# phantomzone-org/fhe-ram

Hardware: AMD Instinct MI355X
Metric: encrypted RAM read ops/s + write ops/s at 2^18 entries; achieved HBM GB/s vs peak (higher is better)
Workload: dtype f64

## Files before the change

fhe-ram_amd/csrc/ctx.hpp:

```cpp
#pragma once
#include "../../include/fheram.h"
#include "kernels.hpp"
#include "cmux_chain.hpp"

#include <algorithm>
#include <atomic>
#include <cstdio>
#include <cstdlib>
#include <cstring>
#include <map>
#include <string>
#include <vector>

using namespace fk;

namespace {

thread_local std::string g_create_err;


struct ProfCls {
    uint64_t launches = 0, blocks = 0;
    double ms = 0.0;
    std::vector<std::pair<hipEvent_t, hipEvent_t>> pending;
};

}

inline uint64_t next_addr_id() { static std::atomic<uint64_t> n{0}; return ++n; }

struct RamState {
    bool initialized = false, state = false;
    bool memo_top = false;
    int memo_alone = 0;
    bool res_in_trtop = false;
};

struct fheram_ctx {
    fheram_params p;
    int device = 0;
    hipStream_t stream = nullptr;
    hipStream_t stream2 = nullptr;
    hipStream_t cur = nullptr;
    hipEvent_t ev_fork = nullptr, ev_join = nullptr;
    hipEvent_t ev_xout = nullptr, ev_xin = nullptr;
    bool side_begun = false;
    bool trhi_in_C = false;
    bool tree_rotate_pending = false;
    int ws = 0, n2 = 0, n_digits = 0;
    size_t rows = 0;
    size_t rows_glob = 0;
    int shard = 0, n_shards = 1;
    std::vector<std::vector<int>> base2d;
    static constexpr int S_CT = 3, S_ADDR = 4, S_INV = 5, DNUM_CT = 3, DNUM_GGSW = 4;
    int s_evk = 4;
    size_t atk = 0;
    static constexpr size_t GLWE = (size_t)S_CT * 2 * N;
    static constexpr size_t GLWE4 = (size_t)S_ADDR * 2 * N;
    static constexpr size_t GGSW = (size_t)DNUM_CT * 2 * GLWE4;
    static constexpr size_t EVK5 = (size_t)DNUM_GGSW * S_INV * 2 * N;
    static constexpr size_t GGSW5 = (size_t)DNUM_GGSW * 2 * S_INV * 2 * N;
    double* d_tw = nullptr;
    double ninv = 0.0;
    double* d_atk = nullptr;
    double* d_atk_inv = nullptr;
    double* d_tsk = nullptr;
    int64_t gal[LOGN];
    bool keys_loaded = false;
    int32_t* d_data = nullptr;
    int32_t* d_tree = nullptr;
    int32_t* d_scrA = nullptr;
    int32_t* d_scrB = nullptr;
    int32_t* d_scrC = nullptr;
    int32_t* d_scrD = nullptr;
    int32_t* d_res = nullptr;
    int32_t* d_tmp = nullptr;
    int32_t* d_tmp2 = nullptr;
    int32_t* d_w = nullptr;
    double* d_big = nullptr;
    double* d_big2 = nullptr;
    int limb_split = 1;
    int chain = 1;
    int chain_y = 3;
    int fine_split = 1;
    int use_graph = 0;
    int32_t* d_part = nullptr;
    int32_t* d_gat[3] = {nullptr, nullptr, nullptr};
    int nco = 0;
    int cus = 256;
    double* d_prep = nullptr;
    bool prep1_ready = false;
    int32_t* d_ggsw_tmp = nullptr;
    int32_t* d_ggsw_tmp2 = nullptr;
    int max_digits = 0;
    RamState ram;
    bool words_staged = false;
    int memo = 1;
    int tail = 1;
    int tail_ep = 1;
    int tail_test = 0;
    unsigned tail_seq = 0;
    int tail_xoff = 0;
    uint64_t tail_launches = 0;
    unsigned* h_tail_fb = nullptr;
    unsigned tail_fb_mark = 0;
    uint64_t tail_launch_mark = 0;
    unsigned* d_tail_sync = nullptr;
    int mid = 2;
    int mid_test = 0;
    unsigned mid_seq = 0;
    uint64_t mid_launches = 0, mid_launch_mark = 0;
    unsigned mid_fb_mark = 0;
    int mid_bad_windows = 0, mid_saved = 0;
    uint64_t mid_window_cts = 0, mid_disabled_count = 0;
    unsigned mid_off_ops = 0;
    unsigned* h_mid_fb = nullptr;
    unsigned* d_mid_sync[2] = {nullptr, nullptr};
    double* d_mid_big[2] = {nullptr, nullptr};
    double* d_mid_y[2] = {nullptr, nullptr};
    int pair_z = 1;
    int fuse = 1;
    bool wide = false;
    int safe = 0;
    int monitor = 1;
    unsigned* h_ro_flag = nullptr;
    int pre_inv = 1;
    uint64_t inv_id[2] = {0, 0};
    double* d_prep_inv = nullptr;
    int32_t* d_ggsw_inv = nullptr;
    hipEvent_t ev_inv[2] = {nullptr, nullptr};
// ... 193 lines not shown
```

fhe-ram_amd/csrc/kernels.hpp:

```cpp
#pragma once
#include "fft_dev.hpp"
#include <type_traits>

namespace fk {

#ifdef FK_STAMP
__device__ unsigned long long g_stamps[192];
#define STAMP(i)                                                                                   \
    do {                                                                                           \
        __builtin_amdgcn_sched_barrier(0);                                                         \
        if (threadIdx.x == 0 && blockIdx.x == 0 && blockIdx.y == 0 && blockIdx.z == 0) {           \
            unsigned long long t_;                                                                 \
            asm volatile("s_memtime %0\n\ts_waitcnt lgkmcnt(0)" : "=s"(t_)::"memory");            \
            g_stamps[i] = t_;                                                                      \
        }                                                                                          \
        __builtin_amdgcn_sched_barrier(0);                                                         \
    } while (0)
#define STAMPZ(i)                                                                                  \
    do {                                                                                           \
        __builtin_amdgcn_sched_barrier(0);                                                         \
        if (threadIdx.x == 0 && blockIdx.x == 0 && blockIdx.y == 0 && (blockIdx.z == 0 || blockIdx.z == 3)) { \
            unsigned long long t_;                                                                 \
            asm volatile("s_memtime %0\n\ts_waitcnt lgkmcnt(0)" : "=s"(t_)::"memory");            \
            g_stamps[(blockIdx.z == 0 ? 128 : 144) + (i)] = t_;                                      \
// ... 1322 lines not shown
                bstage[tid + T * k] = window51(__builtin_floor(__builtin_fma(aa[k] - ab[k], 0.5, 0.5)));
                u[k] = window51(__builtin_floor(__builtin_fma(aa[k] + ab[k], 0.5, 0.5)));
            }
        }
    }
    twiddles_commit(twr, tw, tid);
    double xh[SX][E];
    double od[E], ec[E];
    {
        int sidx = sidx0;
#pragma unroll
        for (int k = 0; k < E; k++) {
            const bool ng = sidx >= N;
            double c = mstage[sidx & (N - 1)];
            const double d2 = take_digit(c);
            const double d1 = take_digit(c);
            const double d0 = cmod17(c);
            xh[2][k] = ng ? -d2 : d2;
            xh[1][k] = ng ? -d1 : d1;
            xh[0][k] = ng ? -d0 : d0;
            double w = 0.0;
            if (co == 0) { const double b = bstage[sidx & (N - 1)]; w = ng ? -b : b; }
            od[k] = w;
            ec[k] = 0.0;
            sidx = (sidx + sstep) & (2 * N - 1);
        }
    }
    OpRegs g[SX];
#pragma unroll
    for (int r = 0; r < SX; r++) load_ops(g[r], ka.key + (long)((r * SK + (SK - 1)) * 2 + co) * N, tid);
    fwd_all<SX>(xh, tw, data, tid);
    auto pair = [&](int j) {
        double acc[2][E];
#pragma unroll
        for (int k = 0; k < E; k++) { acc[0][k] = 0.0; acc[1][k] = 0.0; }
#pragma unroll
        for (int r = 0; r < SX; r++) {
            mac_regs(acc[0], xh[r], g[r]);
            __builtin_amdgcn_sched_barrier(0);
            load_ops(g[r], ka.key + (long)((r * SK + (j - 1)) * 2 + co) * N, tid);
            __builtin_amdgcn_sched_barrier(0);
        }
#pragma unroll
        for (int r = 0; r < SX; r++) mac_regs(acc[1], xh[r], g[r]);
        __builtin_amdgcn_sched_barrier(0);
        ntt_inv2_loop(acc, tw, data, data + LDS_DATA, tid);
        fold_limb<SK>(od, ec, acc[0], j);
        fold_limb<SK>(od, ec, acc[1], j - 1);
        if (j >= 2) {
#pragma unroll
            for (int r = 0; r < SX; r++) load_ops(g[r], ka.key + (long)((r * SK + (j - 2)) * 2 + co) * N, tid);
        }
    };
#pragma unroll 1
    for (int j = SK - 1; j >= 1; j -= 2) pair(j);
    if constexpr (SK & 1) {
        double acc[1][E];
#pragma unroll
        for (int k = 0; k < E; k++) acc[0][k] = 0.0;
#pragma unroll
        for (int r = 0; r < SX; r++) mac_regs(acc[0], xh[r], g[r]);
        ntt_inv1_loop(acc, tw, data, tid);
        fold_limb<SK>(od, ec, acc[0], 0);
    }
#pragma unroll
    for (int k = 0; k < E; k++) {
        double r_ = window51(u[k] - window51(od[k]));
        const double d2 = take_digit(r_);
        const double d1 = take_digit(r_);
        int dst = tid + T * k + ka.t;
        const bool ng = dst >= N;
        if (ng) dst -= N;
        gstore_i32(op + glwe_off(2, co), (unsigned)dst * 4u, cneg((int)d2, ng));
        gstore_i32(op + glwe_off(1, co), (unsigned)dst * 4u, cneg((int)d1, ng));
        gstore_i32(op + glwe_off(0, co), (unsigned)dst * 4u, cneg((int)r_, ng));
    }
}

struct RowChainArgs {
    EpChainArgs ep;
    KsChainArgs ks;
    GlweRef hi, trhi;
    int store_ep = 0;
};
#define FK_READ_CHAIN_ARGS RowChainArgs
#define FK_READ_CHAIN_BATCH 0
#define FK_KS_CHAIN_NAME k_keyswitch_chain
#define FK_READ_CHAIN_NAME k_read_chain
#define FK_VG FK_CHAIN_VGPRS
#include "chain_kernels.inc"
#undef FK_KS_CHAIN_NAME
#undef FK_READ_CHAIN_NAME
#undef FK_VG
#define FK_KS_CHAIN_NAME k_keyswitch_chain_w
#define FK_READ_CHAIN_NAME k_read_chain_w
#define FK_VG FK_WIDE_VGPRS
#include "chain_kernels.inc"
#undef FK_KS_CHAIN_NAME
#undef FK_READ_CHAIN_NAME
#undef FK_VG
#undef FK_READ_CHAIN_ARGS
#undef FK_READ_CHAIN_BATCH
struct RowChainBatchArgs : RowChainArgs {
    long opnd_stride = 0;
    int ws = 1, src_rows = 1;
};
template <typename Args>
__device__ __forceinline__ long batch_opnd_offset(const Args& ra) {
    int y = (int)blockIdx.y;
    asm volatile("" : "+v"(y));
    return (long)(__builtin_amdgcn_readfirstlane(y) / ra.ws) * ra.opnd_stride;
}
__device__ __forceinline__ GlweRef batch_src_row(GlweRef a, const RowChainBatchArgs& ra) {
    int y = (int)blockIdx.y;
    asm volatile("" : "+v"(y));
    y = __builtin_amdgcn_readfirstlane(y);
    a.p += (long)(y % ra.src_rows - y) * a.sy;
    return a;
}
#define FK_READ_CHAIN_ARGS RowChainBatchArgs
#define FK_READ_CHAIN_BATCH 1
#define FK_READ_CHAIN_NAME k_read_chain_b
#define FK_VG FK_CHAIN_VGPRS
#include "chain_kernels.inc"
#undef FK_READ_CHAIN_NAME
#undef FK_VG
#define FK_READ_CHAIN_NAME k_read_chain_bw
#define FK_VG FK_WIDE_VGPRS
#include "chain_kernels.inc"
#undef FK_READ_CHAIN_NAME
#undef FK_VG
#undef FK_READ_CHAIN_ARGS
#undef FK_READ_CHAIN_BATCH
struct RowChainListArgs : RowChainArgs {
    long opnd_stride = 0;
    int ws = 1;
    unsigned src_map = 0;
};
__device__ __forceinline__ GlweRef list_src_row(GlweRef a, const RowChainListArgs& ra) {
    int y = (int)blockIdx.y;
    asm volatile("" : "+v"(y));
    const int k = __builtin_amdgcn_readfirstlane(y) / ra.ws;
    const int m = (int)((ra.src_map >> (4 * k)) & 15u);
    a.p += (long)((m - k) * ra.ws) * a.sy;
    return a;
}
#define FK_READ_CHAIN_ARGS RowChainListArgs
#define FK_READ_CHAIN_BATCH 2
#define FK_READ_CHAIN_NAME k_read_chain_lw
#define FK_VG FK_WIDE_VGPRS
#include "chain_kernels.inc"
#undef FK_READ_CHAIN_NAME
#undef FK_VG
#undef FK_READ_CHAIN_ARGS
#undef FK_READ_CHAIN_BATCH

#define FK_WRITE_CHAIN_ARGS RowChainArgs
#define FK_WRITE_CHAIN_BATCH 0
#define FK_WRITE_CHAIN_NAME k_write_chain
#include "write_chain.inc"
#undef FK_WRITE_CHAIN_ARGS
#undef FK_WRITE_CHAIN_BATCH
#undef FK_WRITE_CHAIN_NAME
#define FK_WRITE_CHAIN_ARGS RowChainBatchArgs
#define FK_WRITE_CHAIN_BATCH 1
#define FK_WRITE_CHAIN_NAME k_write_chain_b
// ... 759 lines not shown
```

fhe-ram_amd/csrc/launch.hpp:

```cpp
#pragma once
#include "ctx.hpp"

namespace {

template <typename F>
void with_evk(const fheram_ctx* c, F&& f) {
    if (c->s_evk == 5) f(std::integral_constant<int, 5>{});
    else f(std::integral_constant<int, 4>{});
}
template <typename F>
void with_evk_wide(fheram_ctx* c, bool wide, F&& f) {
    if (wide) c->wide_unsynced = true;
    with_evk(c, [&](auto sk) { if (wide) f(sk, std::true_type{}); else f(sk, std::false_type{}); });
}
bool capturing(const fheram_ctx* c) { return c->use_graph && !c->profile; }

constexpr int LIMB_SPLIT_MAX = 64;
constexpr int EW_SLICES = 8;
int pick_nco(const fheram_ctx* c, int gx, int gy, bool one_wg = false) {
    if (c->nco != 0) return c->nco;
    if (one_wg) return 2;
    return ((long)gx * gy * 2 <= c->cus) ? 1 : 2;
}
void launch_prepare(fheram_ctx* c, const int32_t* in, double* out, int npoly, int64_t gal = 0) {
// ... 207 lines not shown
    if (d >= 2) hipLaunchKernelGGL((k_ext_product_chain_r<4>), dim3(gx, gy, 1), dim3(T), LDS_BYTES, c->cur, ca);
    else hipLaunchKernelGGL((k_ext_product_chain<3, 4>), dim3(gx, gy, 1), dim3(T), LDS_BYTES, c->cur, ca);
}
void ep_chain(fheram_ctx* c, GlweRef src, GlweRef dst, GlweRef tmp, const double* prep, int d, int gx, int gy) {
    if (gx <= 0 || gy <= 0) return;
    GlweRef b[2];
    bool fits;
    switch (plan_chain(c, ChainQuery{true, d, gx, gy}, src, dst, tmp, b, fits).form) {
    case ChainForm::Mid: launch_mid_ep(c, src, b, prep, d, gx, gy); return;
    case ChainForm::Chain:
        if (!fits && !chain_bufs(d, src, tmp, dst, b)) break;
        launch_ep_chain(c, src, b, prep, d, gx, gy);
        if (!fits) launch_copy(c, tmp, dst, gx, gy);
        return;
    default: break;
    }
    run_chain(c, d, src, dst, tmp, gx, gy, [&](int i, GlweRef in, GlweRef out) { launch_ep(c, in, out, prep + (size_t)i * fheram_ctx::GGSW, gx, gy); });
}
void launch_trace_chain(fheram_ctx* c, GlweRef src, const GlweRef (&b)[2], int start, int n, int gx, int gy, int rot_mul, int rot_base) {
    ProfScope ps(c, "keyswitch", (uint64_t)gx * gy, n);
    ProfScope pf(c, "keyswitch_fused", (uint64_t)gx * gy, n);
    ProfScope pl(c, "keyswitch_chain_launch", (uint64_t)gx * gy * n, 1);
    KsChainArgs ca;
    ca.base = ks_args(c, src, src, b[0], trace_key(c, start), c->gal[start], 0, rot_mul, rot_base);
    ca.buf[0] = b[0]; ca.buf[1] = b[1]; ca.n = n;
    for (int i = 0; i < n; i++) { ca.key[i] = trace_key(c, start + i); ca.ginv[i] = galois_inv_mod(galois_mod(c->gal[start + i])); }
    const int yf = n >= 2 ? c->chain_y : 0;
    with_evk_wide(c, yf && c->wide, [&](auto sk, auto w) {
        constexpr int SK = decltype(sk)::value;
        if (!yf) hipLaunchKernelGGL((k_keyswitch_chain<3, SK, 3>), dim3(gx, gy, 1), dim3(T), LDS_BYTES, c->cur, ca);
        else if constexpr (decltype(w)::value) hipLaunchKernelGGL((k_keyswitch_chain_w<3, SK, 3, 3>), dim3(gx, gy, 1), dim3(T), LDS_BYTES, c->cur, ca);
        else hipLaunchKernelGGL((k_keyswitch_chain<3, SK, 3, 3>), dim3(gx, gy, 1), dim3(T), LDS_BYTES, c->cur, ca);
    });
}
struct OpndTable { int ws = 0; long stride = 0; int src_rows = 0; bool mapped = false; unsigned src_map = 0; };
bool use_row_fuse(const fheram_ctx* c, int d, int n_tr, int gx, int gy, bool one_wg = false) {
    return c->fuse && c->chain_y == 3 && !capturing(c) &&
           chain_form(c, ChainQuery{true, d, gx, gy, false, one_wg}).form == ChainForm::Chain &&
           chain_form(c, ChainQuery{false, n_tr, gx, gy, false, one_wg}).form == ChainForm::Chain;
}
RowChainBatchArgs with_table(const RowChainArgs& ra, const OpndTable& t, int src_rows) {
    RowChainBatchArgs rb;
    static_cast<RowChainArgs&>(rb) = ra;
    rb.opnd_stride = t.stride; rb.ws = t.ws; rb.src_rows = src_rows;
    return rb;
}
void fill_row_chain(fheram_ctx* c, RowChainArgs& ra, const double* prep, int d, int start, int n_tr) {
    ra.ep.tw = c->d_tw; ra.ep.n = d;
    for (int i = 0; i < d; i++) ra.ep.ggsw[i] = prep + (size_t)i * fheram_ctx::GGSW;
    ra.ks.n = n_tr;
    for (int i = 0; i < n_tr; i++) { ra.ks.key[i] = trace_key(c, start + i); ra.ks.ginv[i] = galois_inv_mod(galois_mod(c->gal[start + i])); }
}
void launch_read_chain(fheram_ctx* c, GlweRef src, const GlweRef* ep_store, GlweRef dst, const double* prep, int d, int n_tr, int gx, int gy, const OpndTable& t) {
    ProfScope ps(c, "read_chain_launch", (uint64_t)gx * gy, 1);
    RowChainArgs ra;
    fill_row_chain(c, ra, prep, d, 0, n_tr);
    ra.ep.src = src;
    ra.ep.buf[0] = ra.ep.buf[1] = ep_store ? *ep_store : dst;
    ra.store_ep = ep_store ? 1 : 0;
    ra.ks.base = ks_args(c, dst, dst, dst, trace_key(c, 0), c->gal[0]);
    ra.ks.buf[0] = ra.ks.buf[1] = dst;
    ra.hi = dst; ra.trhi = dst;
    if (t.mapped) {
        RowChainListArgs rl;
        static_cast<RowChainArgs&>(rl) = ra;
        rl.opnd_stride = t.stride; rl.ws = t.ws; rl.src_map = t.src_map;
        c->wide_unsynced = true;
        with_evk(c, [&](auto sk) { hipLaunchKernelGGL((k_read_chain_lw<decltype(sk)::value, 4>), dim3(gx, gy, 1), dim3(T), LDS_BYTES, c->cur, rl); });
        return;
    }
    with_evk_wide(c, c->wide, [&](auto sk, auto w) {
        constexpr int SK = decltype(sk)::value;
        constexpr bool W = decltype(w)::value;
        if (t.ws > 0) {
            const RowChainBatchArgs rb = with_table(ra, t, t.src_rows);
            if constexpr (W) hipLaunchKernelGGL((k_read_chain_bw<SK, 4>), dim3(gx, gy, 1), dim3(T), LDS_BYTES, c->cur, rb);
            else hipLaunchKernelGGL((k_read_chain_b<SK, 4>), dim3(gx, gy, 1), dim3(T), LDS_BYTES, c->cur, rb);
        } else {
            if constexpr (W) hipLaunchKernelGGL((k_read_chain_w<SK, 4>), dim3(gx, gy, 1), dim3(T), LDS_BYTES, c->cur, ra);
            else hipLaunchKernelGGL((k_read_chain<SK, 4>), dim3(gx, gy, 1), dim3(T), LDS_BYTES, c->cur, ra);
        }
    });
}
void launch_write_chain(fheram_ctx* c, GlweRef src, int rot_mul, int rot_base, GlweRef data, GlweRef trhi, const double* prep, int d, int n_tr, int gx, int gy, const OpndTable& t) {
    ProfScope ps(c, "write_chain_launch", (uint64_t)gx * gy, 1);
    RowChainArgs ra;
    fill_row_chain(c, ra, prep, d, 0, n_tr);
    ra.ks.base = ks_args(c, src, src, data, trace_key(c, 0), c->gal[0], 0, rot_mul, rot_base);
    ra.ks.buf[0] = ra.ks.buf[1] = data;
    ra.hi = data; ra.trhi = trhi;
    ra.ep.src = data; ra.ep.buf[0] = ra.ep.buf[1] = data;
    c->wide_unsynced = true;
    with_evk(c, [&](auto sk) {
        constexpr int SK = decltype(sk)::value;
        if (t.ws > 0) hipLaunchKernelGGL((k_write_chain_b<SK, 4>), dim3(gx, gy, 1), dim3(T), LDS_BYTES, c->cur, with_table(ra, t, gy));
        else hipLaunchKernelGGL((k_write_chain<SK, 4>), dim3(gx, gy, 1), dim3(T), LDS_BYTES, c->cur, ra);
    });
}
void launch_trace_tail(fheram_ctx* c, GlweRef src, const GlweRef (&b)[2], int start, int n, int gx, int gy,
                       const double* prep = nullptr, int d = 0, GlweRef ep_out = GlweRef{nullptr, 0, 0}, bool store_ep = false, const OpndTable& t = {}) {
    ProfScope ps(c, "keyswitch", (uint64_t)gx * gy, n);
    ProfScope pt(c, "keyswitch_tail_launch", (uint64_t)gx * gy * n, 1);
    TailArgs ta;
    ta.src = src; ta.buf[0] = b[0]; ta.buf[1] = b[1]; ta.tw = c->d_tw; ta.big = big_of(c); ta.sync = c->d_tail_sync;
    ta.n_ep = prep ? d : 0; ta.ep_out = ep_out;
    for (int i = 0; i < TAIL_EP_MAX; i++) ta.ggsw[i] = (prep && i < d) ? prep + (size_t)i * fheram_ctx::GGSW : nullptr;
    if (++c->tail_seq == 0) ++c->tail_seq;
    c->tail_launches++;
    if (c->tail_test != 1 && c->tail_launches - c->tail_launch_mark >= 64) {
        const unsigned fb = *(volatile unsigned*)c->h_tail_fb;
        if (fb - c->tail_fb_mark > 16) c->tail = 0;
        c->tail_fb_mark = fb;
        c->tail_launch_mark = c->tail_launches;
    }
    ta.seq = c->tail_seq; ta.n = n; ta.n_ct = gx * gy; ta.gx = gx; ta.xoff = c->tail_xoff; ta.give_up_at = c->tail_test ? ta.n_ep + n - 2 : -1;
    KsChainArgs ca;
    ca.base = ks_args(c, src, src, b[0], trace_key(c, start), c->gal[start], 0, 0, 0);
    ca.buf[0] = b[0]; ca.buf[1] = b[1]; ca.n = n;
    ca.pred = c->d_tail_sync + TAIL_GROUPS * 32; ca.pred_seq = ta.seq; ca.host_count = c->h_tail_fb;
    for (int i = 0; i < n; i++) { ta.key[i] = ca.key[i] = trace_key(c, start + i); ta.ginv[i] = ca.ginv[i] = galois_inv_mod(galois_mod(c->gal[start + i])); }
    RowChainArgs ra;
    if (ta.n_ep) {
        fill_row_chain(c, ra, prep, d, start, n);
        ra.ep.src = src; ra.ep.buf[0] = ra.ep.buf[1] = ep_out; ra.store_ep = store_ep ? 1 : 0;
        ra.ks.base = ks_args(c, b[(n - 1) & 1], b[(n - 1) & 1], b[(n - 1) & 1], trace_key(c, start), c->gal[start]);
        ra.ks.buf[0] = ra.ks.buf[1] = b[(n - 1) & 1];
        ra.hi = ra.trhi = b[(n - 1) & 1];
        ra.ks.pred = ca.pred; ra.ks.pred_seq = ca.pred_seq; ra.ks.host_count = ca.host_count;
    }
    with_evk(c, [&](auto sk) {
        constexpr int SK = decltype(sk)::value;
        const dim3 groups(TAIL_GROUPS * 2 * SK * 3);
        if (t.ws > 0 && ta.n_ep) {
            TailBatchArgs tb;
            static_cast<TailArgs&>(tb) = ta;
            tb.opnd_stride = t.stride; tb.ws = t.ws;
            hipLaunchKernelGGL((k_trace_tail_b<3, SK, 3>), groups, dim3(T), LDS_BYTES, c->cur, tb);
            hipLaunchKernelGGL((k_read_chain_b<SK, 4>), dim3(gx, gy, 1), dim3(T), LDS_BYTES, c->cur, with_table(ra, t, gx * gy));
            return;
        }
        hipLaunchKernelGGL((k_trace_tail<3, SK, 3>), groups, dim3(T), LDS_BYTES, c->cur, ta);
        if (ta.n_ep) hipLaunchKernelGGL((k_read_chain<SK, 4>), dim3(gx, gy, 1), dim3(T), LDS_BYTES, c->cur, ra);
        else hipLaunchKernelGGL((k_keyswitch_chain<3, SK, 3>), dim3(gx, gy, 1), dim3(T), LDS_BYTES, c->cur, ca);
    });
}
void trace_steps(fheram_ctx* c, GlweRef src, GlweRef dst, GlweRef tmp, int start, int end, int gx, int gy, int rot_mul = 0, int rot_base = 0) {
    if (gx <= 0 || gy <= 0) return;
    const int n = end - start;
    GlweRef b[2];
    bool fits;
    const ChainPlan p = plan_chain(c, ChainQuery{false, n, gx, gy, rot_mul != 0 || rot_base != 0}, src, dst, tmp, b, fits);
    switch (p.form) {
    case ChainForm::Tail: launch_trace_tail(c, src, b, start, n, gx, gy); return;
    case ChainForm::Mid: launch_mid_trace(c, src, b, start, n, gx, gy, rot_mul, rot_base, p.split); return;
    case ChainForm::Chain:
        if (!fits && !chain_bufs(n, src, tmp, dst, b)) break;
        launch_trace_chain(c, src, b, start, n, gx, gy, rot_mul, rot_base);
        if (!fits) launch_copy(c, tmp, dst, gx, gy);
        return;
    case ChainForm::Steps: break;
    }
    run_chain(c, n, src, dst, tmp, gx, gy, [&](int i, GlweRef in, GlweRef out) {
        KsArgs ka = ks_args(c, in, in, out, trace_key(c, start + i), c->gal[start + i], 0, i == 0 ? rot_mul : 0, i == 0 ? rot_base : 0);
        launch_ks_tr<KS_TRACE>(c, ka, gx, gy);
    });
}
int32_t* pack_levels(fheram_ctx* c, int32_t* src, int32_t* A, int32_t* B, long sy, long sx, size_t count, int gy,
                     int n_alone, int first_pair, bool keep_alone = false, int32_t* P0 = nullptr, int32_t* P1 = nullptr) {
    const int k = ilog2_ceil(count);
    int32_t* cur = src;
    auto other = [&](int32_t* x) { return x == A ? B : A; };
    if (n_alone > 0 && count > 0) {
        int32_t* b0 = other(src);
        int32_t* b1 = other(b0);
        if (b1 == src && P0 && P0 != src && chain_form(c, ChainQuery{false, n_alone, (int)count, gy}).form == ChainForm::Tail) b1 = P0;
        cur = keep_alone ? A : ((n_alone - 1) & 1) ? b1 : b0;
        trace_steps(c, ref(src, sy, sx), ref(cur, sy, sx), ref(cur == b0 ? b1 : b0, sy, sx), 0, n_alone, (int)count, gy);
    }
    size_t live = count;
    for (int m = 0; m < k; m++) {
// ... 65 lines not shown
```

fhe-ram_amd/csrc/path.hpp:

```cpp
#pragma once
#include "launch.hpp"

namespace {

struct Opnds {
    fheram_ctx* c;
    RamState* st;
    const fheram_addr* const* addrs;
    int n, ws;
    double *tab, *tab_inv;
    long stride;
    bool own_rows;
    bool mapped = false;
    unsigned src_map = 0;
    int member(int k) const { return (int)((src_map >> (4 * k)) & 15u); }
    int Y() const { return n * ws; }
    double* prep(int k, int ci) const { return digits_of(c, tab + k * stride, ci); }
    double* inv(int k, int ci) const { return digits_of(c, tab_inv + k * stride, ci); }
    GlweRef slice(GlweRef r, int k) const { r.p += (long)k * ws * r.sy; return r; }
    GlweRef rows(GlweRef r, int k) const { return mapped ? slice(r, member(k)) : own_rows ? slice(r, k) : r; }
    OpndTable table() const { return n == 1 ? OpndTable{} : OpndTable{ws, stride, own_rows ? Y() : ws, mapped, src_map}; }
    bool row_fuse(int d, int n_tr, int gx) const { return use_row_fuse(c, d, n_tr, gx, Y(), n > 1 && (own_rows || mapped)); }
};
Opnds one_addr(fheram_ctx* c, const fheram_addr* const* a, int ws, RamState* st) { return Opnds{c, st, a, 1, ws, c->d_prep, c->d_prep_inv, 0, true}; }
Opnds one_addr(fheram_ctx* c, const fheram_addr* const* a) { return one_addr(c, a, c->ws, &c->ram); }

struct RamView {
    int32_t *rows, *A, *B, *C, *D;
    int32_t *part, *tmp, *tmp2, *res, *tree, *w, *trtop;
};
RamView ctx_view(const fheram_ctx* c) {
    return RamView{c->d_data, c->d_scrA, c->d_scrB, c->d_scrC, c->d_scrD, c->d_part, c->d_tmp, c->d_tmp2, c->d_res, c->d_tree, c->d_w, c->d_trtop};
}

void read_local_done(const fheram_ctx* c, RamState* st, bool prepare_write) {
    if (c->n2 == 2) st->memo_alone = (prepare_write && c->memo) ? LOGN - ilog2_ceil(c->rows_glob) : 0;
}
void read_top_done(fheram_ctx* c, RamState* st, bool prepare_write) {
    st->memo_top = prepare_write && c->memo;
    st->res_in_trtop = st->memo_top;
    c->prep1_ready = false;
}
void write_done(fheram_ctx* c, RamState* st) { st->memo_top = false; st->memo_alone = 0; c->side_begun = false; c->tree_rotate_pending = false; }

template <typename F>
int run_op(fheram_ctx* c, const fheram_addr* addr, int which, F&& enqueue) {
    if (!c->use_graph || c->profile) return enqueue();
    fheram_addr* a = const_cast<fheram_addr*>(addr);
    const unsigned sig = 1u | (c->ram.memo_top ? 2u : 0u) | ((unsigned)c->ram.memo_alone << 2) | (c->side_begun ? 64u : 0u) |
                         (c->inv_id[0] == addr->id ? 128u : 0u) | (c->inv_id[1] == addr->id ? 256u : 0u);
    if (a->graph[which] && a->graph_sig[which] != sig) { hipGraphExecDestroy(a->graph[which]); a->graph[which] = nullptr; }
    if (!a->graph[which]) {
        hipGraph_t g = nullptr;
        HIPCHK(c, hipStreamBeginCapture(c->stream, hipStreamCaptureModeThreadLocal));
        const int rc = enqueue();
        const hipError_t e = hipStreamEndCapture(c->stream, &g);
        if (rc != FHERAM_OK || e != hipSuccess) {
            if (g) hipGraphDestroy(g);
            return rc != FHERAM_OK ? rc : fail(c, FHERAM_ERR_DEVICE, std::string("hipStreamEndCapture: ") + hipGetErrorString(e));
        }
        const hipError_t e2 = hipGraphInstantiate(&a->graph[which], g, nullptr, nullptr, 0);
        hipGraphDestroy(g);
        if (e2 != hipSuccess) { a->graph[which] = nullptr; return fail(c, FHERAM_ERR_DEVICE, std::string("hipGraphInstantiate: ") + hipGetErrorString(e2)); }
        a->graph_sig[which] = sig;
    }
    HIPCHK(c, hipGraphLaunch(a->graph[which], c->stream));
    if (which == 2) write_done(c, &c->ram);
    else { read_local_done(c, &c->ram, which == 1); read_top_done(c, &c->ram, which == 1); }
    return FHERAM_OK;
}

int check_common(fheram_ctx* c, const fheram_addr* addr) {
    if (!c) return FHERAM_ERR_INVALID_ARG;
    mid_rearm(c);
    if (!addr || addr->ctx != c) return fail(c, FHERAM_ERR_INVALID_ARG, "address does not belong to this context (layout mismatch, ram.rs:404)");
    if (addr->empty) return fail(c, FHERAM_ERR_INVALID_ARG, "empty address: fheram_address_alloc without fheram_address_derive");
    if (!c->ram.initialized) return fail(c, FHERAM_ERR_UNINITIALIZED, "unitialized memory: self.data.len()=0");
    if (!c->keys_loaded) return fail(c, FHERAM_ERR_KEYS, "evaluation keys not loaded");
    return FHERAM_OK;
}

int read_local(const Opnds& o, const RamView& a, bool prepare_write, GlweRef* packed_out, bool to_part) {
    fheram_ctx* c = o.c;
    const int n = o.n, ws = o.ws, Y = o.Y(), R = (int)c->rows;
    c->wide = !prepare_write || n > 1;
    if (n == 1 && prepare_write && c->pre_inv == 1 && !capturing(c) && (c->wide_unsynced || c->derive_unsynced)) {
        hipEventRecord(c->ev_opstart, c->stream);
        c->opstart_valid = true;
    }
    const long G = (long)fheram_ctx::GLWE;
    const long sy = (long)c->rows * G;
    GlweRef data = ref(a.rows, sy, G), A = ref(a.A, sy, G), B = ref(a.B, sy, G);
    GlweRef part = ref(a.part, G, 0);
    const bool all = (c->n_shards == 1 && c->n2 == 2);
    for (int k = 0; k < n; k++)
        if (all) coordinate_prepare_all(c, o.addrs[k], o.tab + k * o.stride); else coordinate_prepare(c, o.addrs[k], 0, o.tab + k * o.stride);
    c->prep1_ready = all;
    read_local_done(c, o.st, prepare_write);
    const int d0 = (int)c->base2d[0].size();
    if (c->n2 == 1) {
        GlweRef row0 = ref(a.rows, sy, 0);
        for (int k = 0; k < n; k++)
            if (prepare_write) ep_chain(c, o.rows(row0, k), o.rows(row0, k), o.slice(ref(a.A, sy, 0), k), o.prep(k, 0), d0, 1, ws);
            else ep_chain(c, o.rows(row0, k), o.slice(part, k), o.slice(ref(a.tmp, G, 0), k), o.prep(k, 0), d0, 1, ws);
        *packed_out = prepare_write ? row0 : part;
        if (prepare_write && to_part) launch_copy(c, row0, part, 1, Y);
        return FHERAM_OK;
    }
    const int L0 = LOGN - ilog2_ceil(c->rows_glob);
    const bool keep = o.st->memo_alone > 0;
    int32_t* packed;
    if (o.row_fuse(d0, L0, R) && !(prepare_write && (d0 & 1))) {
        launch_read_chain(c, data, prepare_write ? &data : nullptr, A, o.prep(0, 0), d0, L0, R, Y, o.table());
        packed = pack_levels(c, a.A, a.A, a.B, sy, G, (size_t)R, Y, 0, L0, keep, a.C, a.D);
    } else {
        for (int k = 0; k < n; k++)
            if (prepare_write) ep_chain(c, o.rows(data, k), o.rows(data, k), o.slice(A, k), o.prep(k, 0), d0, R, ws);
            else ep_chain(c, o.rows(data, k), o.slice(A, k), o.slice(B, k), o.prep(k, 0), d0, R, ws);
        packed = pack_levels(c, prepare_write ? a.rows : a.A, a.A, a.B, sy, G, (size_t)R, Y, L0, L0, keep, a.C, a.D);
    }
    *packed_out = ref(packed, sy, 0);
    if (to_part) launch_copy(c, *packed_out, part, 1, Y);
    return FHERAM_OK;
}
int read_top(const Opnds& o, const RamView& a, bool prepare_write, int32_t* gathered, GlweRef pk) {
    fheram_ctx* c = o.c;
// ... 70 lines not shown
bool batch_needs_third(const fheram_ctx* c, int K) { return third_arena_needed(c, K * c->ws); }
int batch_reserve(fheram_ctx* c, int K) {
    const bool third = batch_needs_third(c, K);
    if (K <= c->batch_cap && (!third || c->d_bC)) return FHERAM_OK;
    if (K < c->batch_cap) K = c->batch_cap;
    if (c->batch_cap) { HIPCHK(c, hipStreamSynchronize(c->stream)); batch_free(c); }
    const size_t G = fheram_ctx::GLWE, nct = (size_t)K * c->ws, nrow = nct * c->rows;
    hipError_t e = hipSuccess;
    auto dev = [&](auto** p, size_t bytes) { if (e == hipSuccess) e = hipMalloc((void**)p, bytes); };
    dev(&c->d_bA, nrow * G * sizeof(int32_t));
    dev(&c->d_bB, nrow * G * sizeof(int32_t));
    if (third) dev(&c->d_bC, nrow * G * sizeof(int32_t));
    dev(&c->d_bres, nct * G * sizeof(int32_t));
    dev(&c->d_btmp, nct * G * sizeof(int32_t));
    dev(&c->d_btmp2, nct * G * sizeof(int32_t));
    dev(&c->d_bprep, (size_t)K * c->n_digits * fheram_ctx::GGSW * sizeof(double));
    if (e == hipSuccess) e = hipHostMalloc((void**)&c->h_bres, (nct * G + 1) * sizeof(int64_t), hipHostMallocMapped);
    if (e == hipSuccess) e = hipHostGetDevicePointer((void**)&c->d_h_bres, c->h_bres, 0);
    if (e != hipSuccess) {
        batch_free(c);
        (void)hipGetLastError();
        return fail(c, FHERAM_ERR_DEVICE, std::string("read batch buffers for ") + std::to_string(K) + " addresses: " + hipGetErrorString(e));
    }
    c->batch_cap = K;
    return FHERAM_OK;
}
Opnds batch_opnds(fheram_ctx* c, const fheram_addr* const* addrs, int K) { return Opnds{c, &c->ram, addrs, K, c->ws, c->d_bprep, nullptr, (long)c->n_digits * (long)fheram_ctx::GGSW, false}; }
RamView batch_view(const fheram_ctx* c) { return RamView{c->d_data, c->d_bA, c->d_bB, c->d_bC, nullptr, c->d_btmp2, c->d_btmp, c->d_btmp2, c->d_bres, nullptr, nullptr, nullptr}; }

struct ResRun { const int32_t* src; size_t n; };
int result_export(fheram_ctx* c, const ResRun* runs, int n_runs, int64_t* h, int64_t* d_h, int64_t* out) {
    size_t n = 0;
    for (int i = 0; i < n_runs; i++) {
        const int n4 = (int)(runs[i].n / 4);
        hipLaunchKernelGGL(k_export_i64, dim3((n4 + 255) / 256), dim3(256), 0, c->stream, runs[i].src, reinterpret_cast<long long*>(d_h + n), n4,
                           reinterpret_cast<const long long*>(c->d_tw + N));
        n += runs[i].n;
    }
    HIPCHK(c, hipStreamSynchronize(c->stream));
    HIPCHK(c, hipGetLastError());
    c->wide_unsynced = c->derive_unsynced = false;
    double m;
    std::memcpy(&m, h + n, 8);
    if (c->monitor && m > MON_LIMIT) __atomic_store_n(c->h_ro_flag, 1u, __ATOMIC_RELAXED);
    const int rc = check_precision(c);
    if (rc == FHERAM_OK && out) std::memcpy(out, h, n * sizeof(int64_t));
    return rc;
}

int write_top(const Opnds& o, const RamView& v) {
    fheram_ctx* c = o.c;
    c->wide = true;
    const long G = (long)fheram_ctx::GLWE;
    const long sy = (long)c->rows * G;
    const int n = o.n, ws = o.ws, Y = o.Y();
    GlweRef wref = ref(v.w, G, 0), tmp = ref(v.tmp, G, 0), tmp2 = ref(v.tmp2, G, 0), tree = ref(v.tree, G, 0);
    GlweRef top = (c->n2 != 1) ? tree : ref(v.rows, sy, 0);
    GlweRef tr = tmp;
    if (o.st->memo_top) tr = ref(v.trtop, G, 0);
    else trace_steps(c, top, tmp, tmp2, 0, LOGN, 1, Y);
    {
        ProfScope ps(c, "elementwise", Y);
        hipLaunchKernelGGL((k_sub_add_norm<3>), dim3(1, Y, EW_SLICES), dim3(256), 0, c->cur, top, tr, wref, top);
    }
    o.st->memo_top = false;
    if (c->n2 == 2) {
        if (n == 1 && c->inv_id[1] == o.addrs[0]->id) wait_inverse(c, c->stream, 1);
        else {
            if (n == 1 && c->inv_pending[1]) wait_inverse(c, c->stream, 1);
            for (int k = 0; k < n; k++) coordinate_prepare_inv(c, o.addrs[k], 1, c->d_ggsw_tmp, o.inv(k, 1));
        }
        if (n == 1) { c->inv_pending[1] = false; c->inv_id[1] = 0; }
        for (int k = 0; k < n; k++)
            ep_chain(c, o.slice(tree, k), o.slice(ref(v.part, G, 0), k), o.slice(tmp, k), o.inv(k, 1), (int)c->base2d[1].size(), 1, ws);
        c->tree_rotate_pending = true;
    }
    return FHERAM_OK;
}
void write_side_begin(const Opnds& o, const RamView& v) {
    fheram_ctx* c = o.c;
    c->wide = true;
    const long G = (long)fheram_ctx::GLWE;
    const long sy = (long)c->rows * G;
    hipEventRecord(c->ev_fork, c->stream);
    hipStreamWaitEvent(c->stream2, c->ev_fork, 0);
    c->cur = c->stream2;
    if (c->n2 == 2) {
        const int kept = o.st->memo_alone;
        c->trhi_in_C = kept > 0 && (LOGN - kept) % 2 == 1;
        if (kept > 0) trace_steps(c, ref(v.A, sy, G), ref(c->trhi_in_C ? v.C : v.A, sy, G), ref(c->trhi_in_C ? v.A : v.C, sy, G), kept, LOGN, (int)c->rows, o.Y());
        else trace_steps(c, ref(v.rows, sy, G), ref(v.A, sy, G), ref(v.C, sy, G), 0, LOGN, (int)c->rows, o.Y());
        o.st->memo_alone = 0;
    }
    if (o.n == 1 && c->inv_id[0] == o.addrs[0]->id) wait_inverse(c, c->stream2, 0);
    else for (int k = 0; k < o.n; k++) coordinate_prepare_inv(c, o.addrs[k], 0, c->d_ggsw_tmp2, o.inv(k, 0));
    if (o.n == 1) { c->inv_id[0] = 0; c->inv_pending[0] = false; }
    hipEventRecord(c->ev_join, c->stream2);
    c->cur = c->stream;
    c->side_begun = true;
}
void write_side_abort(fheram_ctx* c) {
    if (!c->side_begun) return;
    hipStreamWaitEvent(c->stream, c->ev_join, 0);
    c->side_begun = false;
}
int write_rows(const Opnds& o, const RamView& v) {
    fheram_ctx* c = o.c;
    c->wide = true;
    const long G = (long)fheram_ctx::GLWE;
    const long sy = (long)c->rows * G;
    const int n = o.n, ws = o.ws, Y = o.Y(), R = (int)c->rows;
    GlweRef data = ref(v.rows, sy, G), A = ref(v.A, sy, G), B = ref(v.B, sy, G), D = ref(v.D, sy, G);
    GlweRef trhi = ref(c->trhi_in_C ? v.C : v.A, sy, G), part = ref(v.part, G, 0);
    const int d0 = (int)c->base2d[0].size();
    const bool fuse = c->n2 == 2 && o.row_fuse(d0, LOGN, R);
    if (fuse) {
        hipStreamWaitEvent(c->stream, c->ev_join, 0);
        launch_write_chain(c, part, c->n_shards, c->shard, data, trhi, o.inv(0, 0), d0, LOGN, R, Y, o.table());
    } else if (c->n2 == 2)
        trace_steps(c, part, B, D, 0, LOGN, R, Y, c->n_shards, c->shard);
    if (c->tree_rotate_pending) {
        ProfScope ps(c, "elementwise", Y);
        hipLaunchKernelGGL((k_rotate<3>), dim3(1, Y, EW_SLICES), dim3(256), 0, c->cur, part, ref(v.tree, G, 0), -(int)c->rows_glob);
    }
    if (!fuse) {
        hipStreamWaitEvent(c->stream, c->ev_join, 0);
        if (c->n2 == 2) {
            ProfScope ps(c, "elementwise", (uint64_t)R * Y);
            hipLaunchKernelGGL((k_sub_add_norm<3>), dim3(R, Y, EW_SLICES), dim3(256), 0, c->cur, data, trhi, B, data);
        }
        for (int k = 0; k < n; k++) ep_chain(c, o.slice(data, k), o.slice(data, k), o.slice(A, k), o.inv(k, 0), d0, R, ws);
    }
    if (n == 1 && !capturing(c)) { hipEventRecord(c->ev_wdone, c->stream); c->wdone_pending = true; }
    write_done(c, o.st);
    o.st->state = false;
    return FHERAM_OK;
}

}
```

fhe-ram_amd/csrc/setup.hpp:

```cpp
#pragma once
#include "launch.hpp"

namespace {
void wipe_free(hipStream_t st, void* d, size_t bytes) {
    if (!d) return;
    if (hipMemsetAsync(d, 0, bytes, st) == hipSuccess) hipStreamSynchronize(st);
    hipFree(d);
}
void wipe_host(void* p, size_t bytes) {
    volatile unsigned char* v = static_cast<volatile unsigned char*>(p);
    for (size_t i = 0; i < bytes; i++) v[i] = 0;
}
}

namespace {

constexpr int64_t NOISE_LIM = (int64_t)1 << 30;
int noise_limb(int k) { return (k + BASE2K - 1) / BASE2K - 1; }

template <int S, int DEC>
void launch_enc(fheram_ctx* c, int32_t* cts, const double* s_hat, const int32_t* pt1, int n) {
    ProfScope ps(c, "encrypt", (uint64_t)n);
    hipLaunchKernelGGL((k_encrypt_sk<S, DEC>), dim3(n), dim3(T), LDS_BYTES, c->cur, cts, s_hat, c->d_tw, pt1);
}
// ... 428 lines not shown
    }
    c->cur = c->stream;
    int digit = 0;
    unsigned bit_rsh = 0;
    for (auto& base1d : c->base2d) {
        unsigned bit_lsh = 0;
        for (int bit_mask : base1d) {
            GlweRef acc = ref(a->d_ggsw + (size_t)digit * fheram_ctx::GGSW, 0, g4);
            GlweRef t = ref(tbuf.p, 0, g4), ev = ref(ebuf.p, 0, g4);
            for (int i = 0; i < bit_mask; i++) {
                const int step = 1 << (i + bit_lsh);
                const double* gb = f->d_prep + (size_t)(bit_rsh + i) * fheram_ctx::GGSW5;
                ProfScope ps(c, "set_from_fheuint", rows);
                hipLaunchKernelGGL((k_cmux_pre<S>), dim3(rows, 1, EW_SLICES), dim3(256), 0, c->cur, acc, t, sign ? step : -step);
                hipLaunchKernelGGL((k_ext_product_fine<S, SG>), dim3(rows, 1, 2 * SG * 2 * S), dim3(T), LDS_BYTES, c->cur, t, gb, c->d_tw, big);
                hipLaunchKernelGGL((k_ext_product_fine_norm<S, SG>), dim3(rows, 1, 2 * (N / 256)), dim3(256), 0, c->cur, ev, big);
                hipLaunchKernelGGL((k_add_norm<S>), dim3(rows, 1, EW_SLICES), dim3(256), 0, c->cur, acc, ev, acc);
            }
            bit_lsh += (unsigned)bit_mask;
            bit_rsh += (unsigned)bit_mask;
            digit++;
        }
    }
    if (e == hipSuccess) e = hipStreamSynchronize(c->stream);
    if (e == hipSuccess) e = hipGetLastError();
    hipFree(big);
    if (e != hipSuccess) { fheram_address_destroy(a); return fail(c, FHERAM_ERR_DEVICE, std::string("set_from_fheuint: ") + hipGetErrorString(e)); }
    *out = a;
    return FHERAM_OK;
}

int fheram_address_alloc(fheram_ctx* c, fheram_addr** out) {
    if (!c || !out) return FHERAM_ERR_INVALID_ARG;
    *out = nullptr;
    HIPCHK(c, hipSetDevice(c->device));
    fheram_addr* a = new fheram_addr{c, nullptr, c->n_digits, c->device};
    a->empty = true;
    const hipError_t e = hipMalloc(&a->d_ggsw, (size_t)c->n_digits * fheram_ctx::GGSW * sizeof(int32_t));
    if (e != hipSuccess) { delete a; return fail(c, FHERAM_ERR_DEVICE, std::string("hipMalloc: ") + hipGetErrorString(e)); }
    *out = a;
    return FHERAM_OK;
}
int fheram_address_derive(fheram_ctx* c, const fheram_fheuint* const* fus, int n, int sign, fheram_addr* const* addrs) {
    if (!c) return FHERAM_ERR_INVALID_ARG;
    if (!fus || !addrs) return fail(c, FHERAM_ERR_INVALID_ARG, "null integer or address list");
    if (n < 1 || n > FHERAM_DERIVE_MAX)
        return fail(c, FHERAM_ERR_INVALID_ARG, "n = " + std::to_string(n) + " is outside [1, FHERAM_DERIVE_MAX = " + std::to_string(FHERAM_DERIVE_MAX) + "]");
    static_assert(FHERAM_DERIVE_MAX == DERIVE_K_MAX, "the argument struct of k_cmux_chain holds FHERAM_DERIVE_MAX integers and addresses");
    unsigned bits = 0;
    for (auto& b1 : c->base2d) for (int b : b1) bits += (unsigned)b;
    for (int k = 0; k < n; k++) {
        if (!fus[k] || fus[k]->ctx != c) return fail(c, FHERAM_ERR_INVALID_ARG, "integer " + std::to_string(k) + " is null or belongs to another context");
        if (!addrs[k] || addrs[k]->ctx != c) return fail(c, FHERAM_ERR_INVALID_ARG, "address " + std::to_string(k) + " is null or belongs to another context");
        if ((int)bits > fus[k]->n_bits) return fail(c, FHERAM_ERR_INVALID_ARG, "the address plan is wider than the encrypted integer");
        for (int q = 0; q < k; q++)
            if (addrs[q] == addrs[k]) return fail(c, FHERAM_ERR_INVALID_ARG, "address " + std::to_string(k) + " appears twice in the list");
    }
    if (c->n_digits > DERIVE_DIGITS_MAX)
        return fail(c, FHERAM_ERR_UNSUPPORTED, "fheram_address_derive takes digit plans of at most " + std::to_string(DERIVE_DIGITS_MAX) + " digits");
    HIPCHK(c, hipSetDevice(c->device));
    CmuxChainArgs ca{};
    ca.tw = c->d_tw;
    ca.sign = sign ? 1 : 0;
    {
        int digit = 0;
        unsigned bit_rsh = 0;
        for (auto& base1d : c->base2d) {
            unsigned bit_lsh = 0;
            for (int bit_mask : base1d) {
                ca.first[digit] = (unsigned char)bit_rsh; ca.bits[digit] = (unsigned char)bit_mask; ca.lsh[digit] = (unsigned char)bit_lsh;
                bit_lsh += (unsigned)bit_mask;
                bit_rsh += (unsigned)bit_mask;
                digit++;
            }
        }
    }
    bool wait_inv[2] = {false, false};
    for (int k = 0; k < n; k++) {
        ca.fu[k] = fus[k]->d_prep;
        ca.out[k] = addrs[k]->d_ggsw;
        for (int ci = 0; ci < 2; ci++) if (c->inv_pending[ci] && c->inv_id[ci] == addrs[k]->id) wait_inv[ci] = true;
    }
    for (int ci = 0; ci < 2; ci++) if (wait_inv[ci]) HIPCHK(c, hipStreamWaitEvent(c->stream, c->ev_inv[ci], 0));
    if (c->side_begun) HIPCHK(c, hipStreamWaitEvent(c->stream, c->ev_join, 0));
    c->cur = c->stream;
    {
        const int rows = fheram_ctx::DNUM_CT * 2;
        ProfScope ps(c, "derive", (uint64_t)n * c->n_digits * rows);
        cmux_chain_launch(dim3(rows, c->n_digits, n), c->cur, ca);
    }
    HIPCHK(c, hipGetLastError());
    for (int k = 0; k < n; k++) { addrs[k]->id = next_addr_id(); addrs[k]->empty = false; }
    c->derive_unsynced = true;
    return FHERAM_OK;
}

}
```

fhe-ram_amd/csrc/write_chain.inc:

```
#if FK_WRITE_CHAIN_BATCH
#define FK_WC_OPND(i) (ra.ep.ggsw[i] + batch_opnd_offset(ra))
#else
#define FK_WC_OPND(i) ra.ep.ggsw[i]
#endif
template <int SK, int SG>
__global__ __launch_bounds__(T, T / 256) __attribute__((amdgpu_num_vgpr(FK_WIDE_VGPRS))) void FK_WRITE_CHAIN_NAME(FK_WRITE_CHAIN_ARGS ra) {
    extern __shared__ __attribute__((aligned(16))) double lds[];
    RoMonitor ro_mon(lds, ra.ep.tw);
    double vc[E];
    KsArgs ka = ra.ks.base;
#pragma unroll 1
    for (int i = 0; i < ra.ks.n; i++) {
        ka.out = ra.ks.buf[i & 1];
        ka.key = ra.ks.key[i];
        ka.ginv = ra.ks.ginv[i];
        int tid = vt((int)threadIdx.x);
        asm volatile("" : "+v"(tid));
        __builtin_assume(tid >= 0 && tid < T);
        if (i == 0) ks_trace_l<SK, false, 1>(ka, lds, true, tid, vc);
        else if (i + 1 < ra.ks.n) ks_trace_l<SK, true, 1>(ka, lds, false, tid, vc);
        else { ka.b = ra.hi; ka.out = ra.trhi; ks_trace_l<SK, true, 2>(ka, lds, false, tid, vc); }
        ka.rot_mul = 0;
        ka.rot_base = 0;
    }
    GlweRef in = ra.ep.src;
#pragma unroll 1
    for (int i = 0; i < ra.ep.n; i++) {
        const GlweRef out = ra.ep.buf[i & 1];
        int tid = vt((int)threadIdx.x);
        asm volatile("" : "+v"(tid));
        __builtin_assume(tid >= 0 && tid < T);
        if (i == 0) ep_step_r<SG, 2, 1>(in, out, FK_WC_OPND(i), ra.ep.tw, lds, false, tid, vc);
        else if (i + 1 < ra.ep.n) ep_step_r<SG, 1, 1>(in, out, FK_WC_OPND(i), ra.ep.tw, lds, false, tid, vc);
        else ep_step_r<SG, 1, 0>(in, out, FK_WC_OPND(i), ra.ep.tw, lds, false, tid, vc);
        in = out;
    }
}
#undef FK_WC_OPND
```

Baseline: 1310.

## Fold trace(ct_hi) steps into fused write chain kernel instead of side stream

When the row-fused write path applies, the trace steps on the high ciphertext that previously ran as separate launches on the side stream are now executed inside the write chain kernel before its own keyswitch trace steps. If the inverse coordinate preparation was already started, the side stream fork is skipped entirely and the main stream waits on the inverse event directly. This removes extra kernel launches and cross-stream synchronization, at the cost of serializing that work onto the main stream and losing overlap with the side-stream work. It also adds validation of n_hi and per-stage profiling counters.

```diff
diff --git a/fhe-ram_amd/csrc/ctx.hpp b/fhe-ram_amd/csrc/ctx.hpp
--- a/fhe-ram_amd/csrc/ctx.hpp
+++ b/fhe-ram_amd/csrc/ctx.hpp
@@ -46,6 +46,8 @@
     hipEvent_t ev_xout = nullptr, ev_xin = nullptr;
     bool side_begun = false;
     bool trhi_in_C = false;
+    int side_n_hi = 0;
+    bool side_forked = false;
     bool tree_rotate_pending = false;
     int ws = 0, n2 = 0, n_digits = 0;
     size_t rows = 0;
diff --git a/fhe-ram_amd/csrc/kernels.hpp b/fhe-ram_amd/csrc/kernels.hpp
--- a/fhe-ram_amd/csrc/kernels.hpp
+++ b/fhe-ram_amd/csrc/kernels.hpp
@@ -1428,6 +1428,7 @@
     KsChainArgs ks;
     GlweRef hi, trhi;
     int store_ep = 0;
+    int n_hi = 0;
 };
 #define FK_READ_CHAIN_ARGS RowChainArgs
 #define FK_READ_CHAIN_BATCH 0
diff --git a/fhe-ram_amd/csrc/launch.hpp b/fhe-ram_amd/csrc/launch.hpp
--- a/fhe-ram_amd/csrc/launch.hpp
+++ b/fhe-ram_amd/csrc/launch.hpp
@@ -313,12 +313,19 @@
         }
     });
 }
-void launch_write_chain(fheram_ctx* c, GlweRef src, int rot_mul, int rot_base, GlweRef data, GlweRef trhi, const double* prep, int d, int n_tr, int gx, int gy, const OpndTable& t) {
+bool launch_write_chain(fheram_ctx* c, GlweRef src, int rot_mul, int rot_base, GlweRef data, GlweRef hi_src, int n_hi, GlweRef trhi, const double* prep, int d, int n_tr, int gx, int gy, const OpndTable& t) {
+    if (n_hi < 0 || n_hi == 1 || n_hi > n_tr || (n_hi && same(trhi, data))) return false;
     ProfScope ps(c, "write_chain_launch", (uint64_t)gx * gy, 1);
+    if (c->profile == 1) {
+        ProfCls &pk = c->prof["write_chain_keyswitch"], &pe = c->prof["write_chain_ext_product"];
+        pk.launches += n_hi + n_tr; pk.blocks += (uint64_t)gx * gy * (n_hi + n_tr);
+        pe.launches += d; pe.blocks += (uint64_t)gx * gy * d;
+    }
     RowChainArgs ra;
     fill_row_chain(c, ra, prep, d, 0, n_tr);
     ra.ks.base = ks_args(c, src, src, data, trace_key(c, 0), c->gal[0], 0, rot_mul, rot_base);
-    ra.ks.buf[0] = ra.ks.buf[1] = data;
+    ra.ks.buf[0] = n_hi ? hi_src : data; ra.ks.buf[1] = data;
+    ra.n_hi = n_hi;
     ra.hi = data; ra.trhi = trhi;
     ra.ep.src = data; ra.ep.buf[0] = ra.ep.buf[1] = data;
     c->wide_unsynced = true;
@@ -327,6 +334,7 @@
         if (t.ws > 0) hipLaunchKernelGGL((k_write_chain_b<SK, 4>), dim3(gx, gy, 1), dim3(T), LDS_BYTES, c->cur, with_table(ra, t, gy));
         else hipLaunchKernelGGL((k_write_chain<SK, 4>), dim3(gx, gy, 1), dim3(T), LDS_BYTES, c->cur, ra);
     });
+    return true;
 }
 void launch_trace_tail(fheram_ctx* c, GlweRef src, const GlweRef (&b)[2], int start, int n, int gx, int gy,
                        const double* prep = nullptr, int d = 0, GlweRef ep_out = GlweRef{nullptr, 0, 0}, bool store_ep = false, const OpndTable& t = {}) {
diff --git a/fhe-ram_amd/csrc/path.hpp b/fhe-ram_amd/csrc/path.hpp
--- a/fhe-ram_amd/csrc/path.hpp
+++ b/fhe-ram_amd/csrc/path.hpp
@@ -41,7 +41,7 @@
     st->res_in_trtop = st->memo_top;
     c->prep1_ready = false;
 }
-void write_done(fheram_ctx* c, RamState* st) { st->memo_top = false; st->memo_alone = 0; c->side_begun = false; c->tree_rotate_pending = false; }
+void write_done(fheram_ctx* c, RamState* st) { st->memo_top = false; st->memo_alone = 0; c->side_begun = false; c->side_n_hi = 0; c->tree_rotate_pending = false; }
 
 template <typename F>
 int run_op(fheram_ctx* c, const fheram_addr* addr, int which, F&& enqueue) {
@@ -278,26 +278,32 @@
     c->wide = true;
     const long G = (long)fheram_ctx::GLWE;
     const long sy = (long)c->rows * G;
+    const int kept = c->n2 == 2 ? o.st->memo_alone : 0;
+    const bool fused = c->n2 == 2 && LOGN - kept >= 2 && o.row_fuse((int)c->base2d[0].size(), LOGN, (int)c->rows);
+    const bool inv_started = o.n == 1 && c->inv_id[0] == o.addrs[0]->id;
+    c->side_n_hi = fused ? LOGN - kept : 0;
+    c->side_forked = !(fused && inv_started);
+    if (c->n2 == 2) o.st->memo_alone = 0;
+    c->side_begun = true;
+    if (!c->side_forked) { c->trhi_in_C = false; return; }
     hipEventRecord(c->ev_fork, c->stream);
     hipStreamWaitEvent(c->stream2, c->ev_fork, 0);
     c->cur = c->stream2;
-    if (c->n2 == 2) {
-        const int kept = o.st->memo_alone;
+    if (fused) c->trhi_in_C = false;
+    else if (c->n2 == 2) {
         c->trhi_in_C = kept > 0 && (LOGN - kept) % 2 == 1;
         if (kept > 0) trace_steps(c, ref(v.A, sy, G), ref(c->trhi_in_C ? v.C : v.A, sy, G), ref(c->trhi_in_C ? v.A : v.C, sy, G), kept, LOGN, (int)c->rows, o.Y());
         else trace_steps(c, ref(v.rows, sy, G), ref(v.A, sy, G), ref(v.C, sy, G), 0, LOGN, (int)c->rows, o.Y());
-        o.st->memo_alone = 0;
-    }
-    if (o.n == 1 && c->inv_id[0] == o.addrs[0]->id) wait_inverse(c, c->stream2, 0);
+    }
+    if (inv_started) wait_inverse(c, c->stream2, 0);
     else for (int k = 0; k < o.n; k++) coordinate_prepare_inv(c, o.addrs[k], 0, c->d_ggsw_tmp2, o.inv(k, 0));
     if (o.n == 1) { c->inv_id[0] = 0; c->inv_pending[0] = false; }
     hipEventRecord(c->ev_join, c->stream2);
     c->cur = c->stream;
-    c->side_begun = true;
 }
 void write_side_abort(fheram_ctx* c) {
     if (!c->side_begun) return;
-    hipStreamWaitEvent(c->stream, c->ev_join, 0);
+    if (c->side_forked) hipStreamWaitEvent(c->stream, c->ev_join, 0);
     c->side_begun = false;
 }
 int write_rows(const Opnds& o, const RamView& v) {
@@ -309,10 +315,14 @@
     GlweRef data = ref(v.rows, sy, G), A = ref(v.A, sy, G), B = ref(v.B, sy, G), D = ref(v.D, sy, G);
     GlweRef trhi = ref(c->trhi_in_C ? v.C : v.A, sy, G), part = ref(v.part, G, 0);
     const int d0 = (int)c->base2d[0].size();
-    const bool fuse = c->n2 == 2 && o.row_fuse(d0, LOGN, R);
+    const int n_hi = c->side_n_hi;
+    const bool fuse = n_hi > 0 || (c->n2 == 2 && o.row_fuse(d0, LOGN, R));
     if (fuse) {
-        hipStreamWaitEvent(c->stream, c->ev_join, 0);
-        launch_write_chain(c, part, c->n_shards, c->shard, data, trhi, o.inv(0, 0), d0, LOGN, R, Y, o.table());
+        if (c->side_forked) hipStreamWaitEvent(c->stream, c->ev_join, 0);
+        else { wait_inverse(c, c->stream, 0); c->inv_id[0] = 0; c->inv_pending[0] = false; }
+        const GlweRef hi_src = n_hi == LOGN ? data : ref(v.A, sy, G);
+        if (!launch_write_chain(c, part, c->n_shards, c->shard, data, hi_src, n_hi, trhi, o.inv(0, 0), d0, LOGN, R, Y, o.table()))
+            return fail(c, FHERAM_ERR_INVALID_ARG, "write chain: no fused form for this number of trace(ct_hi) steps");
     } else if (c->n2 == 2)
         trace_steps(c, part, B, D, 0, LOGN, R, Y, c->n_shards, c->shard);
     if (c->tree_rotate_pending) {
diff --git a/fhe-ram_amd/csrc/setup.hpp b/fhe-ram_amd/csrc/setup.hpp
--- a/fhe-ram_amd/csrc/setup.hpp
+++ b/fhe-ram_amd/csrc/setup.hpp
@@ -534,7 +534,7 @@
         for (int ci = 0; ci < 2; ci++) if (c->inv_pending[ci] && c->inv_id[ci] == addrs[k]->id) wait_inv[ci] = true;
     }
     for (int ci = 0; ci < 2; ci++) if (wait_inv[ci]) HIPCHK(c, hipStreamWaitEvent(c->stream, c->ev_inv[ci], 0));
-    if (c->side_begun) HIPCHK(c, hipStreamWaitEvent(c->stream, c->ev_join, 0));
+    if (c->side_begun && c->side_forked) HIPCHK(c, hipStreamWaitEvent(c->stream, c->ev_join, 0));
     c->cur = c->stream;
     {
         const int rows = fheram_ctx::DNUM_CT * 2;
diff --git a/fhe-ram_amd/csrc/write_chain.inc b/fhe-ram_amd/csrc/write_chain.inc
--- a/fhe-ram_amd/csrc/write_chain.inc
+++ b/fhe-ram_amd/csrc/write_chain.inc
@@ -9,19 +9,26 @@
     RoMonitor ro_mon(lds, ra.ep.tw);
     double vc[E];
     KsArgs ka = ra.ks.base;
+    const int n_hi = ra.n_hi, n_ks = n_hi + ra.ks.n;
 #pragma unroll 1
-    for (int i = 0; i < ra.ks.n; i++) {
-        ka.out = ra.ks.buf[i & 1];
-        ka.key = ra.ks.key[i];
-        ka.ginv = ra.ks.ginv[i];
+    for (int i = 0; i < n_ks; i++) {
+        const int s = i < n_hi ? ra.ks.n - n_hi + i : i - n_hi;
+        ka.out = ra.ks.buf[1];
+        ka.key = ra.ks.key[s];
+        ka.ginv = ra.ks.ginv[s];
         int tid = vt((int)threadIdx.x);
         asm volatile("" : "+v"(tid));
         __builtin_assume(tid >= 0 && tid < T);
-        if (i == 0) ks_trace_l<SK, false, 1>(ka, lds, true, tid, vc);
-        else if (i + 1 < ra.ks.n) ks_trace_l<SK, true, 1>(ka, lds, false, tid, vc);
+        if (i == 0 || i == n_hi) {
+            const bool hi = i < n_hi;
+            ka.a = hi ? ra.ks.buf[0] : ra.ks.base.a;
+            ka.rot_mul = hi ? 0 : ra.ks.base.rot_mul;
+            ka.rot_base = hi ? 0 : ra.ks.base.rot_base;
+            if (i != 0) __syncthreads();
+            ks_trace_l<SK, false, 1>(ka, lds, i == 0, tid, vc);
+        } else if (i + 1 == n_hi) { ka.out = ra.trhi; ks_trace_l<SK, true, 0>(ka, lds, false, tid, vc); }
+        else if (i + 1 < n_ks) ks_trace_l<SK, true, 1>(ka, lds, false, tid, vc);
         else { ka.b = ra.hi; ka.out = ra.trhi; ks_trace_l<SK, true, 2>(ka, lds, false, tid, vc); }
-        ka.rot_mul = 0;
-        ka.rot_base = 0;
     }
     GlweRef in = ra.ep.src;
 #pragma unroll 1
```

New measurement: 1309. No clear change (-0.1%).
